# puzzlepaint/surfelmeshing

Measured on AMD Instinct MI355X. Metric: RGB-D frames/s integrated @640x480, 5M live surfels; achieved HBM GB/s, higher is better.
Workload: dtype f32; 1 GPU; C2: synthetic room stream 640x480, raw depth + colour frames resident in HBM, full preprocessing + Integrate per frame, 4912850 live surfels (6250000 slots), steady-state re-traversal; max_surfel_count=6250000, streams=1, parallelism=1 independent stream per GPU

## Files before the change

surfelmeshing_amd/csrc/smx_recon.hip:

```cpp
#include <math.h>
#include <cmath>
#include <stdlib.h>
#include <string.h>

#include <algorithm>
#include <atomic>
#include <vector>

#include "smx_recon_state.hpp"
#include "smx_mesh.hpp"
#include <hip/hip_ext.h>

using namespace smx;

namespace {

struct FrameCtx {
  Mat34 L;
  Mat34 G;
  float fx, fy, cx, cy;
  Unproj up;
  float inv_depth_scaling;
  float sensor_noise_factor;
  float cos_normal_compat;
// ... 395 lines not shown
        if (vis_bits & (1u << j)) L.vis_list[off++] = i0 + j;
      if (lds_tables) {
#pragma unroll
        for (int j = 0; j < 8; ++j)
          if (key[j] != kNoPair)
            pair_store(tb, key[j], i0 + (uint32_t)(j >> 1),
                       rank[j] != kInvalid ? pair_key[rank[j] >> 16] + (rank[j] & 0xFFFFu) : atomicAdd(&tb.count[(key[j] >> 10) * kCountStride], 1u));
      } else {
#pragma unroll
        for (int j = 0; j < 8; ++j)
          if (key[j] != kNoPair) pair_store(tb, key[j], i0 + (uint32_t)(j >> 1), atomicAdd(&tb.count[(key[j] >> 10) * kCountStride], 1u));
      }
      if (tid == 0) {
        L.vis_seg[seg_id] = total;
        L.seg_act[seg_id] = (total != 0 || box_part[0][7] + box_part[1][7] + box_part[2][7] + box_part[3][7] != 0.0f) ? 1 : 0;
        float lo[3] = {3.0e38f, 3.0e38f, 3.0e38f}, hi[3] = {-3.0e38f, -3.0e38f, -3.0e38f};
        int ns = (int)0x80000000;
        for (int w = 0; w < kBlock / 64; ++w) {
          for (int k = 0; k < 3; ++k) { lo[k] = fminf(lo[k], box_part[w][k]); hi[k] = fmaxf(hi[k], box_part[w][3 + k]); }
          const int o = __float_as_int(box_part[w][6]);
          ns = o > ns ? o : ns;
        }
        box[0] = lo[0]; box[1] = lo[1]; box[2] = lo[2]; box[3] = hi[0]; box[4] = hi[1]; box[5] = hi[2];
        box[6] = __uint_as_float(in_seg);
        box[7] = __int_as_float(ns);
      }
    }
  }
}

template <bool kUseList>
__device__ __forceinline__ uint32_t walk_begin(const Chunks& ch, uint32_t n_slots_scan, uint32_t first, uint32_t& desc, uint32_t& cntv) {
  if (kUseList) {
    desc = ch.desc[(size_t)(first % kSubLists) * ch.stride + first / kSubLists];
    cntv = ch.count[(threadIdx.x % kSubLists) * kCountStride];
    keep(desc); keep(cntv);
    uint32_t longest = cntv;
#pragma unroll
    for (uint32_t off = kSubLists / 2; off > 0; off >>= 1) longest = max(longest, (uint32_t)__shfl_xor((int)longest, (int)off));
    return __builtin_amdgcn_readfirstlane(longest) * kSubLists;
  }
  desc = 0; cntv = 0;
  return (n_slots_scan + kBlock - 1) / kBlock;
}
template <bool kUseList>
__device__ __forceinline__ uint32_t walk_next(const Chunks& ch, uint32_t c, uint32_t n_steps) {
  return (kUseList && c < n_steps) ? ch.desc[(size_t)(c % kSubLists) * ch.stride + c / kSubLists] : 0u;
}
__device__ __forceinline__ bool walk_step_valid(uint32_t c, uint32_t cntv) {
  const uint32_t k = __builtin_amdgcn_readfirstlane(c % kSubLists);
  return c / kSubLists < (uint32_t)__builtin_amdgcn_readlane((int)cntv, (int)k);
}
template <bool kUseList>
__device__ __forceinline__ uint32_t vis_load(const Lists& L, uint32_t c) {
  if (!kUseList) return 0u;
  const uint32_t e = min((c / kSubLists) * (uint32_t)kBlock + threadIdx.x, L.vis_region - 1u);
  return L.vis_list[(size_t)(c % kSubLists) * L.vis_region + e];
}
template <bool kUseList>
__device__ __forceinline__ uint32_t vis_begin(const Lists& L, uint32_t n_slots_scan, uint32_t first, uint32_t& ent, uint32_t& cntv) {
  if (kUseList) {
    ent = vis_load<true>(L, first);
    cntv = L.vis_chunks.count[(threadIdx.x % kSubLists) * kCountStride];
    keep(ent); keep(cntv);
    uint32_t longest = (cntv + (uint32_t)kBlock - 1u) / (uint32_t)kBlock;
#pragma unroll
    for (uint32_t off = kSubLists / 2; off > 0; off >>= 1) longest = max(longest, (uint32_t)__shfl_xor((int)longest, (int)off));
    return __builtin_amdgcn_readfirstlane(longest) * kSubLists;
  }
  ent = 0; cntv = 0;
  return (n_slots_scan + kBlock - 1) / kBlock;
}
template <bool kUseList>
__device__ __forceinline__ bool vis_entry(uint32_t ent, uint32_t c, uint32_t cntv, uint32_t n_slots_scan, uint32_t lane, uint32_t& i) {
  if (kUseList) {
    const uint32_t k = __builtin_amdgcn_readfirstlane(c % kSubLists);
    const uint32_t len = (uint32_t)__builtin_amdgcn_readlane((int)cntv, (int)k);
    i = ent;
    return (c / kSubLists) * (uint32_t)kBlock + lane < len;
  }
  i = c * kBlock + lane;
  return i < n_slots_scan;
}

struct PairRec { uint32_t i, code; Vec3 g, l, gn; float r2; };
__device__ __forceinline__ PairRec fetch_pair(const Surfels& S, const FrameCtx& c, uint32_t i, uint32_t code) {
  const float4 p4 = *S.group(kGroupP, i), n4 = *S.group(kGroupN, i);
  PairRec r;
  r.i = i; r.code = code;
  r.g = Vec3{p4.x, p4.y, p4.z};
  r.l = mul(c.L, r.g);
  r.gn = Vec3{n4.x, n4.y, n4.z};
  r.r2 = n4.w;
  return r;
}
struct TileLds {
  int zmin[kTilePx];
  uint32_t sup[kTilePx], cnt[kTilePx], confl[kTilePx];
  unsigned long long sum[kTilePx];
  float2 nrm[kTilePx];
  uint16_t depth[kTilePx];
};
__device__ __forceinline__ void assoc_stage(TileLds& t, const FrameCtx& c, const PairRec& r) {
  if (!(r.code & kPairActive)) return;
  const uint32_t k = r.code & 255u;
  const float measurement_depth = c.inv_depth_scaling * (float)t.depth[k];
  if (measurement_depth <= 0) return;
  const float first = __int_as_float(t.zmin[k]);
  if (first < (1 - c.sensor_noise_factor) * measurement_depth) {
    if (first == r.l.z) atomicMin(&t.confl[k], 0x80000000u | r.i);
    return;
  }
  const float occlusion_depth = (1 + c.sensor_noise_factor) * measurement_depth;
  if (r.l.z > occlusion_depth) return;
  const float surfel_distance = sqrtf(r.l.x * r.l.x + r.l.y * r.l.y + r.l.z * r.l.z);
  const Vec3 ln = rotate(c.L, r.gn);
  const float dot_angle = (1.0f / surfel_distance) * (r.l.x * ln.x + r.l.y * ln.y + r.l.z * ln.z);
  if (dot_angle > 0) return;
  if (measurement_depth < r.l.z) {
    const float2 n = t.nrm[k];
    const float nz = meas_normal_z(n.x, n.y);
    const float d = ln.x * n.x + ln.y * n.y + ln.z * nz;
    if (d < c.cos_normal_compat) return;
  }
  if (r.r2 <= 0) return;
  atomicMin(&t.sup[k], r.i);
  atomicAdd(&t.cnt[k], 1u);
  atomicAdd(&t.sum[k], (unsigned long long)q_from_float(r.l.z));
}
__device__ __forceinline__ uint32_t merge_candidate(TileLds& t, const FrameCtx& c, const PairRec& r) {
  if (r.code & kPairSecond) return kInvalid;
  if (!(r.r2 >= 0)) return kInvalid;
  const uint32_t k = r.code & 255u;
  const float measurement_depth = c.inv_depth_scaling * (float)t.depth[k];
  if (measurement_depth <= 0) return kInvalid;
  const float first = __int_as_float(t.zmin[k]);
  if (first < (1 - c.sensor_noise_factor) * measurement_depth) {
    if (first == r.l.z) atomicMin(&t.confl[k], r.i);
    return kInvalid;
  }
  const float occlusion_depth = (1 + c.sensor_noise_factor) * measurement_depth;
  if (r.l.z > occlusion_depth) return kInvalid;
  const float surfel_distance = sqrtf(r.l.x * r.l.x + r.l.y * r.l.y + r.l.z * r.l.z);
  const Vec3 ln = rotate(c.L, r.gn);
  const float dot_angle = (1.0f / surfel_distance) * (r.l.x * ln.x + r.l.y * ln.y + r.l.z * ln.z);
  if (dot_angle > 0) return kInvalid;
  if (measurement_depth < r.l.z) {
    const float2 n = t.nrm[k];
    const float nz = meas_normal_z(n.x, n.y);
    const float d = ln.x * n.x + ln.y * n.y + ln.z * nz;
    if (d < c.cos_normal_compat) return kInvalid;
  }
  const uint32_t s = t.sup[k];
  if (s == r.i || s == kInvalid) return kInvalid;
  return s;
}
__device__ __forceinline__ void merge_decide(const PairRec& r, const float4& sp4, const float4& sn4, uint8_t* __restrict__ merge_flag) {
  const float other_r2 = sn4.w;
  const float radius_diff = r.r2 / other_r2;
  const float kT = 1.2f * 1.2f;
  if (radius_diff > kT || radius_diff < 1 / kT) return;
  const float dx = r.g.x - sp4.x, dy = r.g.y - sp4.y, dz = r.g.z - sp4.z;
  const float d2 = dx * dx + dy * dy + dz * dz;
  const float kDist = 0.5f * (0.25f * 0.25f);
  if (d2 > kDist * (r.r2 + other_r2)) return;
  const float dot_angle = r.gn.x * sn4.x + r.gn.y * sn4.y + r.gn.z * sn4.z;
// ... 537 lines not shown
                                                      bool integrate, int x, int y,
                                                      const Vec3& cam, uint32_t i, DevState* st) {
  if (!integrate) return;
  const float measurement_depth = c.inv_depth_scaling * (float)px.depth;
  if (measurement_depth <= 0) return;
  bool conflicting = false;
  const float first = px.first;
  if (first < (1 - c.sensor_noise_factor) * measurement_depth) {
    if (first == cam.z) {
      const uint32_t key = px.key;
      if (key != kInvalid && (key & 0x7FFFFFFFu) == i) conflicting = true;
    }
    integrate = false;
  }
  if (!integrate && !conflicting) return;
  const float occlusion_depth = (1 + c.sensor_noise_factor) * measurement_depth;
  if (cam.z > occlusion_depth) integrate = false;
  if (!integrate && !conflicting) return;

  const float depth = measurement_depth;
  const Vec3 lp = {depth * (c.up.fx_inv * (float)x + c.up.cx_inv), depth * (c.up.fy_inv * (float)y + c.up.cy_inv), depth};
  const Vec3 gp = mul(c.G, lp);
  const float2 nxy = px.nxy;
  const Vec3 mn = {nxy.x, nxy.y, meas_normal_z(nxy.x, nxy.y)};
  const Vec3 gn = rotate(c.G, mn);
  const uchar3 col = px.col;

  if (conflicting) {
    if (c.stats) atomicAdd(&st->n_conflict_hits, 1u);
    float confidence = R.C.x;
    confidence -= 1;
    R.dirty = true;
    if (confidence <= 0) {
      if (c.stats) atomicAdd(&st->n_replaced, 1u);
      R.P = make_float4(gp.x, gp.y, gp.z, __uint_as_float(c.frame));
      R.new_smooth = gp;
      R.replaced = true;
      R.N = make_float4(gn.x, gn.y, gn.z, px.radius);
      R.C = make_float4(1.0f, __uint_as_float(c.frame),
                        __uint_as_float((uint32_t)col.x | ((uint32_t)col.y << 8) | ((uint32_t)col.z << 16) | (1u << 24)), R.C.w);
    } else {
      R.C.x = confidence;
    }
  }
  if (!integrate) return;

  const float surfel_distance = sqrtf(cam.x * cam.x + cam.y * cam.y + cam.z * cam.z);
  const Vec3 sn = {R.N.x, R.N.y, R.N.z};
  const Vec3 ln = rotate(c.L, sn);
  const float dot_angle = (1.0f / surfel_distance) * (cam.x * ln.x + cam.y * ln.y + cam.z * ln.z);
  if (dot_angle > 0) return;
  if (measurement_depth < cam.z) {
    const float d = sn.x * gn.x + sn.y * gn.y + sn.z * gn.z;
    if (d < c.cos_normal_compat) integrate = false;
  }
  const float old_r2 = R.N.w;
  if (old_r2 < 0) integrate = false;
  if (!integrate) return;

  uint32_t cnt = px.count;
  if (cnt < 1) cnt = 1;
  const float weight = 1.0f / (float)cnt;
  if (__float_as_uint(R.C.y) < c.frame) {
    if (c.stats) atomicAdd(&st->n_integrated, 1u);
    const float confidence = R.C.x;
    R.C.x = (confidence + weight < c.max_conf) ? (confidence + weight) : c.max_conf;
    const float nf = 1.0f / (confidence + weight);
    R.P.x = (confidence * R.P.x + weight * gp.x) * nf;
    R.P.y = (confidence * R.P.y + weight * gp.y) * nf;
    R.P.z = (confidence * R.P.z + weight * gp.z) * nf;
    const Vec3 nn = {confidence * sn.x + weight * gn.x, confidence * sn.y + weight * gn.y, confidence * sn.z + weight * gn.z};
    const float inv = 1.0f / sqrtf(nn.x * nn.x + nn.y * nn.y + nn.z * nn.z);
    R.N = make_float4(inv * nn.x, inv * nn.y, inv * nn.z, fminf(old_r2, px.radius));
    const uint32_t oc = __float_as_uint(R.C.z);
    const uint32_t c0 = (uint32_t)(uint8_t)(int)((confidence * (float)(oc & 255u) + weight * (float)col.x) * nf + 0.5f);
    const uint32_t c1 = (uint32_t)(uint8_t)(int)((confidence * (float)((oc >> 8) & 255u) + weight * (float)col.y) * nf + 0.5f);
    const uint32_t c2 = (uint32_t)(uint8_t)(int)((confidence * (float)((oc >> 16) & 255u) + weight * (float)col.z) * nf + 0.5f);
    R.C.z = __uint_as_float(c0 | (c1 << 8) | (c2 << 16));
    R.P.w = __uint_as_float(c.frame);
    R.dirty = true;
  }
}

template <bool kUseList>
__global__ void __launch_bounds__(kBlock)
k_integrate(Surfels S, FrameCtx c, Scratch sc, FrameIn in, Lists L,
            uint8_t* __restrict__ merge_flag, DevState* st, NewFlagsArgs nf, uint32_t n_flag_blocks) {
  SMX_SET_WAVE_PRIO();
#ifdef SMX_STAMPS
  if (nf.dbg && blockIdx.x == 0 && threadIdx.x == 0) nf.dbg[0] = wall_clock64();
#endif
  if (blockIdx.x < n_flag_blocks) { ts_begin(c.ts, kTsIntBegin); new_flags_scan_body(nf, sc, c.W, c.H, st, blockIdx.x); return; }
  const uint32_t block = blockIdx.x - n_flag_blocks, n_blocks = gridDim.x - n_flag_blocks;
  const uint32_t n_scan = kUseList ? 0u : st->surfel_count;
  uint32_t merged_here = 0;
  uint32_t ent, cntv;
  const uint32_t n_steps = vis_begin<kUseList>(L, n_scan, block, ent, cntv);
  for (uint32_t w = block; w < n_steps; w += n_blocks) {
    const uint32_t cur = ent;
    ent = (w + n_blocks < n_steps) ? vis_load<kUseList>(L, w + n_blocks) : 0u;
    uint32_t i;
    if (!vis_entry<kUseList>(cur, w, cntv, n_scan, threadIdx.x, i)) continue;
    const uint32_t merge_mark = merge_flag[i];
    SurfelRegs R;
    R.P = *S.group(kGroupP, i); R.N = *S.group(kGroupN, i); R.C = *S.group(kGroupC, i);
    if (merge_mark) {
      merge_flag[i] = 0;
      S.u(kLastUpdateStamp, i) = 0;
      S.f(kRadiusSq, i) = -1;
      const uint32_t col = (__float_as_uint(R.C.z) & 0x00FFFFFFu) | 0x01000000u;
      S.u(kColor, i) = col;
      L.flags8[i] = make_flags(0u, col, c.frame, c.reg_window);
      L.hot_epoch[i >> L.hot_shift] = (uint8_t)L.epoch;
      if (L.dirty8) L.dirty8[i] = 1;
      ++merged_here;
      continue;
    }
    R.dirty = false; R.replaced = false;
    const float4 p4 = R.P, n4 = R.N;
    if (!is_active(__float_as_uint(p4.w), c.frame, c.window)) continue;
    Proj p;
    const Vec3 g = {p4.x, p4.y, p4.z};
    if (!project_pos(g, c, p)) continue;
    if (n4.w < 0) continue;
    int ox = p.px, oy = p.py;
    const bool second = quadrant(p, c, ox, oy);
    const PixelIn px0 = load_pixel(c, sc, in, p.px, p.py);
    const PixelIn px1 = load_pixel(c, sc, in, ox, oy);
    integrate_or_conflict(R, c, px0, true, p.px, p.py, p.l, i, st);
    integrate_or_conflict(R, c, px1, second, ox, oy, p.l, i, st);
    if (R.dirty) {
      L.hot_epoch[i >> L.hot_shift] = (uint8_t)L.epoch;
      if (L.dirty8) L.dirty8[i] = 1;
      out_store16(S.group(kGroupP, i), R.P); out_store16(S.group(kGroupN, i), R.N);
      out_store16(S.group(kGroupC, i), R.C);
      if (R.replaced) {
        *S.group(kGroupS, i) = make_float4(R.new_smooth.x, R.new_smooth.y, R.new_smooth.z, 0.0f);
        S.set_neighbors(i, make_uint4(kInvalid, kInvalid, kInvalid, kInvalid));
      }
    }
    L.flags8[i] = make_flags(__float_as_uint(R.P.w), __float_as_uint(R.C.z), c.frame, c.reg_window);
  }
#pragma unroll
  for (int off = 32; off > 0; off >>= 1) merged_here += __shfl_xor(merged_here, off);
  if ((threadIdx.x & 63) == 0 && merged_here) {
    atomicAdd(&st->merge_count, merged_here);
    if (c.stats) atomicAdd(&st->n_merged, merged_here);
  }
  ts_end(c.ts, kTsIntEnd, block, min(n_blocks, n_steps));
}

template <bool kUseList>
__device__ __forceinline__ void update_neighbors_body(const Surfels& S, const FrameCtx& c, const Scratch& sc, const FrameIn& in,
                                                      const Lists& L, const DevState* st, uint32_t block, uint32_t n_blocks) {
  const int kDX[4] = {-1, 1, 0, 0}, kDY[4] = {0, 0, -1, 1};
  const uint32_t n_scan = kUseList ? 0u : st->create_base_next;
  if (block == 0 && threadIdx.x < kSubLists) { L.rec_chunks.count[threadIdx.x * kCountStride] = 0; L.acc_chunks.count[threadIdx.x * kCountStride] = 0; }
  uint32_t ent, cntv;
  const uint32_t n_steps = vis_begin<kUseList>(L, n_scan, block, ent, cntv);
  for (uint32_t w = block; w < n_steps; w += n_blocks) {
    const uint32_t cur = ent;
    ent = (w + n_blocks < n_steps) ? vis_load<kUseList>(L, w + n_blocks) : 0u;
    uint32_t i;
    if (!vis_entry<kUseList>(cur, w, cntv, n_scan, threadIdx.x, i)) continue;
    const float4 p4 = *S.group(kGroupP, i), n4 = *S.group(kGroupN, i);
    const uint4 t4 = *reinterpret_cast<const uint4*>(S.group(kGroupT, i));
    if (!is_active(__float_as_uint(p4.w), c.frame, c.window)) continue;
    const Vec3 g = {p4.x, p4.y, p4.z};
    const Vec3 cam = mul(c.L, g);
    if (!(cam.z > 0)) continue;
    const float u = c.fx * (cam.x / cam.z) + c.cx, v = c.fy * (cam.y / cam.z) + c.cy;
    if (!(u >= 1.0f && v >= 1.0f && u < (float)(c.W - 1) && v < (float)(c.H - 1))) continue;
    const int x = (int)u, y = (int)v;
    const float measurement_depth = c.inv_depth_scaling * (float)in.depth(y, x);
    const float obs_r2 = in.radius(y, x);
    uint32_t cand[4];
#pragma unroll
    for (int d = 0; d < 4; ++d) cand[d] = sc.supporting[(size_t)(y + kDY[d]) * c.W + (x + kDX[d])];
    const float occlusion_depth = (1 + c.sensor_noise_factor) * measurement_depth;
    if (cam.z > occlusion_depth) continue;
    const float surfel_distance = sqrtf(cam.x * cam.x + cam.y * cam.y + cam.z * cam.z);
    const Vec3 gn = {n4.x, n4.y, n4.z};
    const Vec3 ln = rotate(c.L, gn);
    const float dot_angle = (1.0f / surfel_distance) * (cam.x * ln.x + cam.y * ln.y + cam.z * ln.z);
    if (dot_angle > 0) continue;
    const float r2 = n4.w;
    if (r2 < 0) continue;
    if (obs_r2 / r2 > 1.5f * 1.5f) continue;

    uint32_t ni[4] = {t4.x, t4.y, t4.z, t4.w};
    float4 np4[4], cp4[4], cn4[4];
#pragma unroll
    for (int q = 0; q < 4; ++q) np4[q] = *S.group(kGroupP, ni[q] == kInvalid ? i : ni[q]);
#pragma unroll
    for (int d = 0; d < 4; ++d) {
      const uint32_t gidx = (cand[d] == kInvalid) ? i : cand[d];
      cp4[d] = *S.group(kGroupP, gidx);
      cn4[d] = *S.group(kGroupN, gidx);
    }
    float nd2[4];
#pragma unroll
    for (int q = 0; q < 4; ++q) {
      if (ni[q] == kInvalid) nd2[q] = __builtin_inff();
      else {
        const float dx = g.x - np4[q].x, dy = g.y - np4[q].y, dz = g.z - np4[q].z;
        nd2[q] = dx * dx + dy * dy + dz * dz;
      }
    }
#pragma unroll
    for (int d = 0; d < 4; ++d) {
      const uint32_t nb = cand[d];
      if (nb == kInvalid || nb == i) continue;
      const float dx = cp4[d].x - g.x, dy = cp4[d].y - g.y, dz = cp4[d].z - g.z;
      const float d2 = dx * dx + dy * dy + dz * dz;
      if (d2 > c.rf2 * r2) continue;
      const float nd = gn.x * cn4[d].x + gn.y * cn4[d].y + gn.z * cn4[d].z;
      if (nd <= 0) continue;
      int best_n = -1; float best_d2 = -1;
#pragma unroll
      for (int q = 0; q < 4; ++q) {
        if (best_n == -2) continue;
        if (nb == ni[q]) { best_n = -2; }
        else if (nd2[q] > best_d2) { best_n = q; best_d2 = nd2[q]; }
      }
      if (best_n >= 0 && d2 < best_d2) {
#pragma unroll
        for (int q = 0; q < 4; ++q) if (q == best_n) { ni[q] = nb; nd2[q] = d2; }
      }
    }
    if (ni[0] != t4.x || ni[1] != t4.y || ni[2] != t4.z || ni[3] != t4.w) {
      S.set_neighbors(i, make_uint4(ni[0], ni[1], ni[2], ni[3]));
      L.hot_epoch[i >> L.hot_shift] = (uint8_t)L.epoch;
    }
  }
  ts_end(c.ts, kTsUpdEnd, block, min(n_blocks, n_steps));
}

struct CreateArgs {
  const uint8_t* flags; const uint32_t* ranks; const uint32_t* block_sums; uint32_t* block_offsets_out;
  int n_scan_blocks; uint32_t max_surfels; uint8_t* flags8; uint8_t* dirty8;
  uint32_t* next_vis_chunk_count;
  int n_pixels;
  uint8_t* hot_epoch; uint32_t epoch; int hot_shift;
};
__device__ __forceinline__ void new_create_body(const Surfels& S, const FrameCtx& c, const Scratch& sc, const FrameIn& in,
                                                const CreateArgs& a, DevState* st, uint32_t block, uint32_t n_blocks) {
  const uint8_t* __restrict__ flags = a.flags;
  const uint32_t* __restrict__ ranks = a.ranks;
  const uint32_t* __restrict__ block_sums = a.block_sums;
  uint32_t* __restrict__ block_offsets_out = a.block_offsets_out;
  const int n_scan_blocks = a.n_scan_blocks;
  const uint32_t max_surfels = a.max_surfels;
  uint8_t* __restrict__ flags8 = a.flags8;
  extern __shared__ uint32_t block_offsets[];
  __shared__ uint32_t wave_tot[kBlock / 64];
  static_assert(kScanPxPerBlock % kBlock == 0, "a creating workgroup's pixels lie inside one scan block");
  if (block != 0 && n_blocks * (uint32_t)kBlock >= (uint32_t)(c.W * c.H) &&
      block_sums[(block * (uint32_t)kBlock) / (uint32_t)kScanPxPerBlock] == 0) return;
  const int per = (n_scan_blocks + kBlock - 1) / kBlock;
  const uint32_t base = st->create_base_next;
  uint32_t mine = 0, total;
  if (per <= 8) {
    uint32_t v[8];
#pragma unroll
    for (int j = 0; j < 8; ++j) {
      const int bidx = threadIdx.x * per + j;
      v[j] = (j < per && bidx < n_scan_blocks) ? block_sums[bidx] : 0u;
    }
#pragma unroll
    for (int j = 0; j < 8; ++j) mine += v[j];
    uint32_t run = block_excl_scan(mine, wave_tot, total);
#pragma unroll
    for (int j = 0; j < 8; ++j) {
      const int bidx = threadIdx.x * per + j;
      if (j < per && bidx < n_scan_blocks) { block_offsets[bidx] = run; run += v[j]; }
    }
  } else {
    for (int j = 0; j < per; ++j) {
      const int bidx = threadIdx.x * per + j;
      if (bidx < n_scan_blocks) mine += block_sums[bidx];
    }
    uint32_t run = block_excl_scan(mine, wave_tot, total);
    for (int j = 0; j < per; ++j) {
      const int bidx = threadIdx.x * per + j;
      if (bidx < n_scan_blocks) { block_offsets[bidx] = run; run += block_sums[bidx]; }
    }
  }
  __syncthreads();
  const uint32_t room = max_surfels - base;
  const uint32_t created = total < room ? total : room;
  if (block == 0) {
    for (int bidx = threadIdx.x; bidx < n_scan_blocks; bidx += kBlock) block_offsets_out[bidx] = block_offsets[bidx];
    if (threadIdx.x == 0) {
      st->create_base = base;
      st->new_count = created;
// ... 877 lines not shown
namespace smx {

int join_regularizer(smx_recon r, hipStream_t st) {
  if (r->reg_pending) {
    SMX_HIP(hipEventRecord(r->ev_reg, r->reg_stream));
    SMX_HIP(hipStreamWaitEvent(st, r->ev_reg, 0));
    if (st == r->last_stream) r->pending_mark = nullptr;
  }
  return SMX_OK;
}

int read_surfel_count(smx_recon r, hipStream_t st, uint32_t* n) {
  SMX_HIP(hipMemcpyAsync(n, &r->st->surfel_count, sizeof(*n), hipMemcpyDeviceToHost, st));
  SMX_HIP(hipStreamSynchronize(st));
  return SMX_OK;
}

void enqueue_segment_scan(hipStream_t st, uint32_t* seg_count, int nseg, uint32_t* total_out) {
  hipLaunchKernelGGL(k_delta_scan, dim3(1), dim3(1024), 0, st, seg_count, nseg, total_out);
}

int acquire_staging(smx_recon r, hipStream_t st, size_t floats) {
  if (r->staging_busy) SMX_HIP(hipStreamWaitEvent(st, r->ev_staging, 0));
  return ensure_staging(r, floats);
}
int release_staging(smx_recon r, hipStream_t st) {
  SMX_HIP(hipEventRecord(r->ev_staging, st));
  r->staging_busy = true;
  return SMX_OK;
}

int invalidate_derived(smx_recon r, hipStream_t st) {
  SMX_HIP(hipMemsetAsync(r->L.vis_seg, 0, (size_t)r->nseg * 4, st));
  SMX_HIP(hipMemsetAsync(r->L.seg_box, 0, (size_t)r->nseg * 8 * sizeof(float), st));
  SMX_HIP(hipMemsetAsync(r->L.recent_seg, 0, (size_t)r->nsegB * 4, st));
  SMX_HIP(hipMemsetAsync(r->vis_count_set[0], 0, sizeof(uint32_t) * kSubLists * kCountStride, st));
  SMX_HIP(hipMemsetAsync(r->vis_count_set[1], 0, sizeof(uint32_t) * kSubLists * kCountStride, st));
  SMX_HIP(hipMemsetAsync(r->L.rec_chunks.count, 0, sizeof(uint32_t) * kSubLists * kCountStride, st));
  hipLaunchKernelGGL(k_rebuild_flags, dim3(r->grid_surfels), dim3(kBlock), 0, st, r->S, 0u, 0x7FFFFFFF, r->L.flags8, r->st);
  SMX_LAUNCH_CHECK();
  r->table_valid = false;
  r->hot_holdoff = 3;
  r->have_frame = false;
  return SMX_OK;
}

}

extern "C" {

int smx_recon_create(uint32_t max_surfel_count, int32_t width, int32_t height,
                     float fx, float fy, float cx, float cy, int32_t device_id, smx_recon* out) {
  SMX_CHECK_ARG(out != nullptr && max_surfel_count > 0 && max_surfel_count <= (1u << 30));
  SMX_CHECK_ARG(width >= 3 && height >= 3);
  int device = 0;
  SMX_CALL(resolve_device(device_id, &device));
  SMX_ON_DEVICE(device);
  {
    static std::atomic<int> advised{0};
    char text[512];
    if (!advised.exchange(1) && smx_runtime_advice(text, sizeof(text)) > 0) {
      const char* quiet = getenv("SMX_QUIET");
      if (!(quiet && quiet[0] == '1')) fprintf(stderr, "libsmx: %s\n", text);
    }
  }
  smx_recon_s* r = new smx_recon_s();
  r->device = device;
  r->max_surfels = max_surfel_count;
  r->W = width; r->H = height; r->fx = fx; r->fy = fy; r->cx = cx; r->cy = cy;
  r->S.pitch = ((size_t)max_surfel_count + 63) / 64 * 64;
  const size_t P = (size_t)width * height;
  int rc;
#define SMX_TRY(x) do { rc = (x); if (rc != SMX_OK) { (void)smx_recon_destroy(r); return rc; } } while (0)
  SMX_TRY(r->mem.alloc(&r->S.base, (size_t)kQuadsPerSlot * 4 * r->S.pitch, true));
  SMX_TRY(r->mem.alloc(&r->grad_acc, 2 * ((size_t)r->S.pitch + kSegAcc), true));
  SMX_TRY(r->mem.alloc(&r->reg_rec, 2 * ((size_t)r->S.pitch + kSegAcc), true));
  r->nseg = div_up((long long)r->S.pitch, kSeg);
  r->nsegB = div_up((long long)r->S.pitch, kSegB);
  r->fb.cap = kFarBinCap; r->fb.hash_mask = (uint32_t)kFarHash - 1u;
  SMX_TRY(r->mem.alloc(&r->fb.rec, (size_t)r->nsegB * kFarBinCap, false));
  SMX_TRY(r->mem.alloc(&r->fb.count, ((size_t)r->nsegB + 1) * kCountStride, true));
  r->L.vis_region = (uint32_t)(div_up(r->nseg, kSubLists) * kSeg);
  SMX_TRY(r->mem.alloc(&r->L.vis_list, (size_t)kSubLists * r->L.vis_region, true));
  SMX_TRY(r->mem.alloc(&r->L.recent_list, (size_t)r->nsegB * kSegB, false));
  SMX_TRY(r->mem.alloc(&r->L.vis_seg, (size_t)r->nseg, true));
  SMX_TRY(r->mem.alloc(&r->L.seg_box, (size_t)r->nseg * 8, true));
  SMX_TRY(r->mem.alloc(&r->L.seg_act, (size_t)r->nseg, true));
  SMX_TRY(r->mem.alloc(&r->L.seg_streak, (size_t)r->nseg, true));
  SMX_TRY(r->mem.alloc(&r->sw.surv_list, (size_t)r->nseg + 65536, true));
  SMX_TRY(r->mem.alloc(&r->sw.copy_list, (size_t)r->nseg + 65536, true));
  SMX_TRY(r->mem.alloc(&r->sw.count, 2, true));
  SMX_TRY(r->mem.alloc_host(&r->dir_host, 2, true));
  r->dir_host[0] = 0;
  r->dir_host[1] = 0;
  SMX_TRY(hip_rc(hipHostGetDevicePointer(reinterpret_cast<void**>(&r->dir_dev), r->dir_host, 0), "hipHostGetDevicePointer"));
  SMX_TRY(r->mem.alloc(&r->L.recent_seg, (size_t)r->nsegB, true));
  r->L.vis_chunks.stride = 0; r->L.vis_chunks.desc = nullptr;
  r->L.rec_chunks.stride = (uint32_t)(div_up(r->nsegB, kSubLists) + 8192);
  SMX_TRY(r->mem.alloc(&r->L.rec_chunks.desc, (size_t)kSubLists * r->L.rec_chunks.stride, true));
  SMX_TRY(r->mem.alloc(&r->L.rec_chunks.count, (size_t)kSubLists * kCountStride, true));
  static_assert(kSegAcc == kSegB && kAccCount < kCountStride, "pass B lists the edge kernel's segments by its own segment numbers");
  r->L.acc_chunks.stride = r->L.rec_chunks.stride;
  r->L.acc_chunks.count = r->L.rec_chunks.count + kAccCount;
  SMX_TRY(r->mem.alloc(&r->L.acc_chunks.desc, (size_t)kSubLists * r->L.acc_chunks.stride, true));
  SMX_TRY(r->mem.alloc(&r->flags_buf[0], (size_t)r->nsegB * kSegB, true));
  SMX_TRY(r->mem.alloc(&r->flags_buf[1], (size_t)r->nsegB * kSegB, true));
  r->L.flags8 = r->flags_buf[0];
  r->L.hot_shift = 10;
  while ((((size_t)r->nseg * kSeg) >> r->L.hot_shift) + 1 > (size_t)kMaxHotGroups) ++r->L.hot_shift;
  r->L.n_hot_groups = (uint32_t)((((size_t)r->nseg * kSeg) >> r->L.hot_shift) + 1);
  SMX_TRY(r->mem.alloc(&r->L.hot_epoch, (size_t)r->L.n_hot_groups + 64, true));
  SMX_TRY(r->mem.alloc(&r->L.seg_targets, (size_t)r->nsegB * kBlockB, true));
  r->L.epoch = 128;
  r->hot_filter_enabled = 1;
  r->fuse_edges = kFuseEdgesDefault;
  r->hot_holdoff = 3;
  SMX_TRY(r->mem.alloc(&r->merge_flag, r->S.pitch, true));
  SMX_TRY(r->mem.alloc(&r->gate_count, 32, true));
  r->gate_expected = 0;
  constexpr int kHandoverModeDefault = 1;
  r->handover_mode = kHandoverModeDefault;
  {
    const char* cc = getenv("ROCPROF_COUNTER_COLLECTION");
    if (cc && cc[0] && strcmp(cc, "0") != 0) r->handover_mode = 0;
  }
  SMX_TRY(r->mem.alloc(&r->L.act_list, (size_t)r->nsegB * kSegB, true));
  SMX_TRY(r->mem.alloc(&r->sc.supporting, P, true));
  SMX_TRY(r->mem.alloc(&r->sc.counts, P, true));
  SMX_TRY(r->mem.alloc(&r->sc.depth_sums, P, true));
  SMX_TRY(r->mem.alloc(&r->sc.confl_key, P, true));
  SMX_TRY(r->mem.alloc(&r->sc.first_depth, P, true));
  for (int k = 0; k < 2; ++k) {
    SMX_TRY(r->mem.alloc(&r->vis_count_set[k], (size_t)kSubLists * kCountStride, true));
    SMX_TRY(r->mem.alloc(&r->ovf_count_set[k], 1, true));
  }
  r->L.vis_chunks.count = r->vis_count_set[0];
  r->tb.tiles_x = div_up(width, kTileW);
  r->tb.n_tiles = (uint32_t)(r->tb.tiles_x * div_up(height, kTileH));
  r->tb.cap = r->bin_cap_full = kTileBinCap;
  SMX_TRY(r->mem.alloc(&r->tb.pairs, (size_t)r->tb.n_tiles * kTileBinCap, false));
  SMX_TRY(r->mem.alloc(&r->tb.count, (size_t)r->tb.n_tiles * kCountStride, true));
  SMX_TRY(r->mem.alloc(&r->tb.ovf, 2 * (size_t)r->S.pitch + 64, false));
  r->tb.ovf_count = r->ovf_count_set[0];
#ifdef SMX_STAMPS
  SMX_TRY(r->mem.alloc(&r->stamps, (size_t)3 * 16 * 8192, true));
#endif
  SMX_TRY(r->mem.alloc(&r->blended_depth, P, true));
  SMX_TRY(r->mem.alloc(&r->bb.distance_map, P, true));
  SMX_TRY(r->mem.alloc(&r->bb.new_distance_map, P, true));
  SMX_TRY(r->mem.alloc(&r->bb.deltas, P, true));
  SMX_TRY(r->mem.alloc(&r->bb.new_deltas, P, true));
  SMX_TRY(r->mem.alloc(&r->new_flags, P, true));
  SMX_TRY(r->mem.alloc(&r->new_ranks, P, true));
  SMX_TRY(r->mem.alloc(&r->tmp_u32, P, true));
  r->n_scan_blocks = div_up((long long)P, kScanPxPerBlock);
  SMX_TRY(r->mem.alloc(&r->block_sums, (size_t)r->n_scan_blocks, true));
  SMX_TRY(r->mem.alloc(&r->block_offsets, (size_t)r->n_scan_blocks, true));
  SMX_TRY(r->mem.alloc(&r->st, 1, true));
  SMX_TRY(r->mem.alloc(&r->ts_ring, (size_t)kTsRing * kTsWords, true));
  SMX_TRY(r->mem.alloc_host(&r->ts_host, (size_t)kTsRing * kTsWords, false));
  SMX_TRY(r->mem.alloc_host(&r->ts_mapped, (size_t)kTsRing * kTsWords, true));
  memset(const_cast<unsigned long long*>(r->ts_mapped), 0, sizeof(unsigned long long) * kTsRing * kTsWords);
  SMX_TRY(hip_rc(hipHostGetDevicePointer(reinterpret_cast<void**>(&r->ts_mapped_dev), const_cast<unsigned long long*>(r->ts_mapped), 0), "hipHostGetDevicePointer"));
  SMX_TRY(hip_rc(hipDeviceGetAttribute(&r->wall_khz, hipDeviceAttributeWallClockRate, device), "hipDeviceGetAttribute"));
  if (r->wall_khz <= 0) r->wall_khz = 100000;
  for (int i = 0; i < 14; ++i) SMX_TRY(hip_rc(hipEventCreate(&r->ev[i]), "hipEventCreate"));
// ... 613 lines not shown
```

surfelmeshing_amd/csrc/smx_recon_state.hpp:

```cpp
#pragma once

#include "smx_common.hpp"

namespace smx {

struct TrackDev;
struct TrackRgbdDev;
struct MeshWorkspace;

enum : int {
  kX = 0, kY = 1, kZ = 2, kSmoothX = 3, kSmoothY = 4, kSmoothZ = 5, kConfidence = 6, kRadiusSq = 7,
  kNormalX = 8, kNormalY = 9, kNormalZ = 10, kGradX = 11, kGradY = 12, kGradZ = 13,
  kCreationStamp = 17, kLastUpdateStamp = 18, kNeighbor0 = 19, kGradCount = 23, kColor = 24, kRows = 25
};

struct DevState {
  uint32_t surfel_count;
  uint32_t merge_count;
  uint32_t create_base_next;
  uint32_t recent_count;
  uint32_t create_base;
  uint32_t new_count;
  uint32_t capacity_clamped;
  uint32_t n_visible, n_merged, n_edges, n_integrated, n_replaced, n_conflict_hits;
  uint32_t n_window_edges, n_contributors;
  uint32_t n_segments_skipped;
  uint32_t reg_saturated;
  uint32_t n_pairs, n_overflow_pairs, max_tile_pairs;
};

enum : int { kGroupP = 0, kGroupS, kGroupN, kGroupT, kGroupC, kGroupG, kGroups };
__host__ __device__ constexpr int row_group(int row) {
  return row <= 2 ? kGroupP : row <= 5 ? kGroupS : row == 6 ? kGroupC : row == 7 ? kGroupN : row <= 10 ? kGroupN
       : row <= 13 ? kGroupG : row <= 16 ? -1 : row == 17 ? kGroupC : row == 18 ? kGroupP : row <= 22 ? kGroupT
       : row == 24 ? kGroupC : -1;
}
__host__ __device__ constexpr int row_sub(int row) {
  return row <= 2 ? row : row <= 5 ? row - 3 : row == 6 ? 0 : row == 7 ? 3 : row <= 10 ? row - 8
       : row <= 13 ? row - 11 : row == 17 ? 1 : row == 18 ? 3 : row <= 22 ? row - 19 : row == 24 ? 2 : -1;
}
__host__ __device__ constexpr int group_start(int g) { return g; }
constexpr int kQuadsPerSlot = 6;
struct Surfels {
  float* base;
  size_t pitch;
  __host__ __device__ __forceinline__ size_t quad(int g, uint32_t i) const { return (size_t)group_start(g) * pitch + (size_t)i; }
  __device__ __forceinline__ float& f(int row, uint32_t i) const { return base[quad(row_group(row), i) * 4 + row_sub(row)]; }
  __device__ __forceinline__ uint32_t& u(int row, uint32_t i) const {
    return reinterpret_cast<uint32_t*>(base)[quad(row_group(row), i) * 4 + row_sub(row)];
  }
  __device__ __forceinline__ float4* group(int g, uint32_t i) const { return reinterpret_cast<float4*>(base) + quad(g, i); }
  __device__ __forceinline__ void set_neighbors(uint32_t i, const uint4& t) const { *reinterpret_cast<uint4*>(group(kGroupT, i)) = t; }
  __device__ __forceinline__ void set_neighbor(uint32_t i, int q, uint32_t v) const { u(kNeighbor0 + q, i) = v; }
};

struct Scratch {
  uint32_t* supporting;
  uint32_t* counts;
  long long* depth_sums;
  uint32_t* confl_key;
  float* first_depth;
};

constexpr int kBlock = 256;

constexpr int kSeg = 1024;
constexpr int kSegB = 1024;
constexpr int kBlockB = kSegB / 4;
constexpr uint32_t kCountStride = 32;
constexpr uint32_t kSubLists = 16;
struct Chunks { uint32_t* desc; uint32_t* count; uint32_t stride; };
struct Lists {
  Chunks vis_chunks, rec_chunks;
  Chunks acc_chunks;
  uint32_t* vis_list;
  uint32_t vis_region;
  float* seg_box;
  uint32_t* vis_seg;
  uint8_t* seg_streak;
  uint32_t* recent_list;
  uint32_t* recent_seg;
  uint32_t* act_list;
  uint8_t* flags8;
  uint8_t* dirty8;
  uint8_t* seg_act;
  uint32_t descending;
  uint8_t* hot_epoch;
  uint16_t* seg_targets;
  uint32_t n_hot_groups;
  uint32_t epoch;
  int hot_shift;
};

struct FarBins {
  uint4* rec;
  uint32_t* count;
  uint32_t cap;
  uint32_t hash_mask;
};

struct TileBins {
  uint2* pairs;
  uint32_t* count;
  uint4* ovf;
  uint32_t* ovf_count;
  uint32_t cap;
  int tiles_x;
  uint32_t n_tiles;
};

template <int kWaves = kBlock / 64>
__device__ __forceinline__ uint32_t block_excl_scan(uint32_t mine, uint32_t* wave_tot , uint32_t& total) {
  const uint32_t lane = threadIdx.x & 63, wave = threadIdx.x >> 6;
  uint32_t incl = mine;
#pragma unroll
  for (int off = 1; off < 64; off <<= 1) {
    const uint32_t t = __shfl_up(incl, off);
    if (lane >= (uint32_t)off) incl += t;
  }
  if (lane == 63) wave_tot[wave] = incl;
  __syncthreads();
  uint32_t wave_off = 0;
  total = 0;
#pragma unroll
  for (int w = 0; w < kWaves; ++w) {
    if ((uint32_t)w < wave) wave_off += wave_tot[w];
    total += wave_tot[w];
  }
  return wave_off + incl - mine;
}

struct BlendBufs {
  uint8_t* distance_map; uint8_t* new_distance_map; float* deltas; float* new_deltas;
};

struct SegWork {
  uint32_t* surv_list;
  uint32_t* copy_list;
  uint32_t* count;
};

}

struct smx_recon_s {
  smx::DevBlocks mem;
  int device;
  uint32_t max_surfels;
  int W, H;
  float fx, fy, cx, cy;
  smx::Surfels S;
  long long* grad_acc;
  float4* reg_rec;
  smx::FarBins fb;
  smx::Lists L;
  int nseg;
  int nsegB;
  uint8_t* merge_flag;
  bool table_valid;
  uint32_t table_frame;
// ... 103 lines not shown
```

Baseline: 6109 frames/s.

## Precompute neighbor-update pixel in integrate and reuse it in update_neighbors

The integrate kernel now evaluates the update_neighbors projection and occlusion/angle/radius tests for each visible-list entry and writes the resulting pixel index (or a no-update sentinel) into a new per-entry upd_px buffer. In list mode, update_neighbors prefetches that word and skips rejected entries early, reading supporting candidates directly from the stored pixel. It also drops candidates that already match the surfel or its current neighbors before loading neighbor data. This trades an extra 4-byte store per entry in integrate for fewer reads of input depth/radius and less ALU in update_neighbors. The tests in integrate use the post-integration surfel state, which is the same state update_neighbors would read afterwards.

Result: no change. 6105 frames/s (-0.1%).

```diff
diff --git a/surfelmeshing_amd/csrc/smx_recon.hip b/surfelmeshing_amd/csrc/smx_recon.hip
--- a/surfelmeshing_amd/csrc/smx_recon.hip
+++ b/surfelmeshing_amd/csrc/smx_recon.hip
@@ -501,6 +501,15 @@
   i = c * kBlock + lane;
   return i < n_slots_scan;
 }
+constexpr uint32_t kNoUpdate = 0xFFFFFFFFu;
+__device__ __forceinline__ uint32_t upd_px_load(const Lists& L, uint32_t c) {
+  const uint32_t e = min((c / kSubLists) * (uint32_t)kBlock + threadIdx.x, L.vis_region - 1u);
+  return L.upd_px[(size_t)(c % kSubLists) * L.vis_region + e];
+}
+__device__ __forceinline__ void upd_px_store(const Lists& L, uint32_t c, uint32_t word) {
+  const uint32_t e = (c / kSubLists) * (uint32_t)kBlock + threadIdx.x;
+  if (e < L.vis_region) L.upd_px[(size_t)(c % kSubLists) * L.vis_region + e] = word;
+}
 
 struct PairRec { uint32_t i, code; Vec3 g, l, gn; float r2; };
 __device__ __forceinline__ PairRec fetch_pair(const Surfels& S, const FrameCtx& c, uint32_t i, uint32_t code) {
@@ -1204,6 +1213,31 @@
   }
 }
 
+__device__ __forceinline__ bool update_pixel(const float4& p4, const FrameCtx& c, Vec3& cam, int& x, int& y) {
+  if (!is_active(__float_as_uint(p4.w), c.frame, c.window)) return false;
+  const Vec3 g = {p4.x, p4.y, p4.z};
+  cam = mul(c.L, g);
+  if (!(cam.z > 0)) return false;
+  const float u = c.fx * (cam.x / cam.z) + c.cx, v = c.fy * (cam.y / cam.z) + c.cy;
+  if (!(u >= 1.0f && v >= 1.0f && u < (float)(c.W - 1) && v < (float)(c.H - 1))) return false;
+  x = (int)u; y = (int)v;
+  return true;
+}
+__device__ __forceinline__ bool update_tests(const Vec3& cam, const float4& n4, const FrameCtx& c, uint16_t depth, float obs_r2) {
+  const float measurement_depth = c.inv_depth_scaling * (float)depth;
+  const float occlusion_depth = (1 + c.sensor_noise_factor) * measurement_depth;
+  if (cam.z > occlusion_depth) return false;
+  const float surfel_distance = sqrtf(cam.x * cam.x + cam.y * cam.y + cam.z * cam.z);
+  const Vec3 gn = {n4.x, n4.y, n4.z};
+  const Vec3 ln = rotate(c.L, gn);
+  const float dot_angle = (1.0f / surfel_distance) * (cam.x * ln.x + cam.y * ln.y + cam.z * ln.z);
+  if (dot_angle > 0) return false;
+  const float r2 = n4.w;
+  if (r2 < 0) return false;
+  if (obs_r2 / r2 > 1.5f * 1.5f) return false;
+  return true;
+}
+
 template <bool kUseList>
 __global__ void __launch_bounds__(kBlock)
 k_integrate(Surfels S, FrameCtx c, Scratch sc, FrameIn in, Lists L,
@@ -1218,11 +1252,12 @@
   uint32_t merged_here = 0;
   uint32_t ent, cntv;
   const uint32_t n_steps = vis_begin<kUseList>(L, n_scan, block, ent, cntv);
+  const auto no_update = [&](uint32_t w) { if (kUseList) upd_px_store(L, w, kNoUpdate); };
   for (uint32_t w = block; w < n_steps; w += n_blocks) {
     const uint32_t cur = ent;
     ent = (w + n_blocks < n_steps) ? vis_load<kUseList>(L, w + n_blocks) : 0u;
     uint32_t i;
-    if (!vis_entry<kUseList>(cur, w, cntv, n_scan, threadIdx.x, i)) continue;
+    if (!vis_entry<kUseList>(cur, w, cntv, n_scan, threadIdx.x, i)) { no_update(w); continue; }
     const uint32_t merge_mark = merge_flag[i];
     SurfelRegs R;
     R.P = *S.group(kGroupP, i); R.N = *S.group(kGroupN, i); R.C = *S.group(kGroupC, i);
@@ -1236,15 +1271,16 @@
       L.hot_epoch[i >> L.hot_shift] = (uint8_t)L.epoch;
       if (L.dirty8) L.dirty8[i] = 1;
       ++merged_here;
+      no_update(w);
       continue;
     }
     R.dirty = false; R.replaced = false;
     const float4 p4 = R.P, n4 = R.N;
-    if (!is_active(__float_as_uint(p4.w), c.frame, c.window)) continue;
+    if (!is_active(__float_as_uint(p4.w), c.frame, c.window)) { no_update(w); continue; }
     Proj p;
     const Vec3 g = {p4.x, p4.y, p4.z};
-    if (!project_pos(g, c, p)) continue;
-    if (n4.w < 0) continue;
+    if (!project_pos(g, c, p)) { no_update(w); continue; }
+    if (n4.w < 0) { no_update(w); continue; }
     int ox = p.px, oy = p.py;
     const bool second = quadrant(p, c, ox, oy);
     const PixelIn px0 = load_pixel(c, sc, in, p.px, p.py);
@@ -1262,6 +1298,14 @@
       }
     }
     L.flags8[i] = make_flags(__float_as_uint(R.P.w), __float_as_uint(R.C.z), c.frame, c.reg_window);
+    if (kUseList) {
+      FrameCtx ct = c;
+      asm volatile("" : "+s"(ct.W), "+s"(ct.H), "+s"(ct.sensor_noise_factor));
+      Vec3 cam; int x = 0, y = 0;
+      bool ok = update_pixel(R.P, ct, cam, x, y);
+      if (ok) ok = update_tests(cam, R.N, ct, in.depth(y, x), in.radius(y, x));
+      upd_px_store(L, w, ok ? (uint32_t)(y * ct.W + x) : kNoUpdate);
+    }
   }
 #pragma unroll
   for (int off = 32; off > 0; off >>= 1) merged_here += __shfl_xor(merged_here, off);
@@ -1279,37 +1323,40 @@
   const uint32_t n_scan = kUseList ? 0u : st->create_base_next;
   if (block == 0 && threadIdx.x < kSubLists) { L.rec_chunks.count[threadIdx.x * kCountStride] = 0; L.acc_chunks.count[threadIdx.x * kCountStride] = 0; }
   uint32_t ent, cntv;
+  uint32_t upd = kUseList ? upd_px_load(L, block) : 0u;
   const uint32_t n_steps = vis_begin<kUseList>(L, n_scan, block, ent, cntv);
+  keep(upd);
   for (uint32_t w = block; w < n_steps; w += n_blocks) {
-    const uint32_t cur = ent;
-    ent = (w + n_blocks < n_steps) ? vis_load<kUseList>(L, w + n_blocks) : 0u;
+    const uint32_t cur = ent, cur_upd = upd;
+    const bool more = w + n_blocks < n_steps;
+    ent = more ? vis_load<kUseList>(L, w + n_blocks) : 0u;
+    upd = (kUseList && more) ? upd_px_load(L, w + n_blocks) : 0u;
     uint32_t i;
     if (!vis_entry<kUseList>(cur, w, cntv, n_scan, threadIdx.x, i)) continue;
+    if (kUseList && cur_upd == kNoUpdate) continue;
     const float4 p4 = *S.group(kGroupP, i), n4 = *S.group(kGroupN, i);
     const uint4 t4 = *reinterpret_cast<const uint4*>(S.group(kGroupT, i));
-    if (!is_active(__float_as_uint(p4.w), c.frame, c.window)) continue;
+    uint32_t cand[4];
+    if (kUseList) {
+#pragma unroll
+      for (int d = 0; d < 4; ++d) cand[d] = sc.supporting[(size_t)((int)cur_upd + kDY[d] * c.W + kDX[d])];
+    } else {
+      Vec3 cam; int x, y;
+      if (!update_pixel(p4, c, cam, x, y)) continue;
+      const uint16_t depth = in.depth(y, x);
+      const float obs_r2 = in.radius(y, x);
+#pragma unroll
+      for (int d = 0; d < 4; ++d) cand[d] = sc.supporting[(size_t)(y + kDY[d]) * c.W + (x + kDX[d])];
+      if (!update_tests(cam, n4, c, depth, obs_r2)) continue;
+    }
     const Vec3 g = {p4.x, p4.y, p4.z};
-    const Vec3 cam = mul(c.L, g);
-    if (!(cam.z > 0)) continue;
-    const float u = c.fx * (cam.x / cam.z) + c.cx, v = c.fy * (cam.y / cam.z) + c.cy;
-    if (!(u >= 1.0f && v >= 1.0f && u < (float)(c.W - 1) && v < (float)(c.H - 1))) continue;
-    const int x = (int)u, y = (int)v;
-    const float measurement_depth = c.inv_depth_scaling * (float)in.depth(y, x);
-    const float obs_r2 = in.radius(y, x);
-    uint32_t cand[4];
-#pragma unroll
-    for (int d = 0; d < 4; ++d) cand[d] = sc.supporting[(size_t)(y + kDY[d]) * c.W + (x + kDX[d])];
-    const float occlusion_depth = (1 + c.sensor_noise_factor) * measurement_depth;
-    if (cam.z > occlusion_depth) continue;
-    const float surfel_distance = sqrtf(cam.x * cam.x + cam.y * cam.y + cam.z * cam.z);
     const Vec3 gn = {n4.x, n4.y, n4.z};
-    const Vec3 ln = rotate(c.L, gn);
-    const float dot_angle = (1.0f / surfel_distance) * (cam.x * ln.x + cam.y * ln.y + cam.z * ln.z);
-    if (dot_angle > 0) continue;
     const float r2 = n4.w;
-    if (r2 < 0) continue;
-    if (obs_r2 / r2 > 1.5f * 1.5f) continue;
-
+
+#pragma unroll
+    for (int d = 0; d < 4; ++d)
+      if (cand[d] == i || cand[d] == t4.x || cand[d] == t4.y || cand[d] == t4.z || cand[d] == t4.w) cand[d] = kInvalid;
+    if ((cand[0] & cand[1] & cand[2] & cand[3]) == kInvalid) continue;
     uint32_t ni[4] = {t4.x, t4.y, t4.z, t4.w};
     float4 np4[4], cp4[4], cn4[4];
 #pragma unroll
@@ -1332,7 +1379,7 @@
 #pragma unroll
     for (int d = 0; d < 4; ++d) {
       const uint32_t nb = cand[d];
-      if (nb == kInvalid || nb == i) continue;
+      if (nb == kInvalid) continue;
       const float dx = cp4[d].x - g.x, dy = cp4[d].y - g.y, dz = cp4[d].z - g.z;
       const float d2 = dx * dx + dy * dy + dz * dz;
       if (d2 > c.rf2 * r2) continue;
@@ -2376,6 +2423,7 @@
   SMX_TRY(r->mem.alloc(&r->fb.count, ((size_t)r->nsegB + 1) * kCountStride, true));
   r->L.vis_region = (uint32_t)(div_up(r->nseg, kSubLists) * kSeg);
   SMX_TRY(r->mem.alloc(&r->L.vis_list, (size_t)kSubLists * r->L.vis_region, true));
+  SMX_TRY(r->mem.alloc(&r->L.upd_px, (size_t)kSubLists * r->L.vis_region, true));
   SMX_TRY(r->mem.alloc(&r->L.recent_list, (size_t)r->nsegB * kSegB, false));
   SMX_TRY(r->mem.alloc(&r->L.vis_seg, (size_t)r->nseg, true));
   SMX_TRY(r->mem.alloc(&r->L.seg_box, (size_t)r->nseg * 8, true));
diff --git a/surfelmeshing_amd/csrc/smx_recon_state.hpp b/surfelmeshing_amd/csrc/smx_recon_state.hpp
--- a/surfelmeshing_amd/csrc/smx_recon_state.hpp
+++ b/surfelmeshing_amd/csrc/smx_recon_state.hpp
@@ -75,6 +75,7 @@
   Chunks acc_chunks;
   uint32_t* vis_list;
   uint32_t vis_region;
+  uint32_t* upd_px;
   float* seg_box;
   uint32_t* vis_seg;
   uint8_t* seg_streak;
```
